# imulki/serenade

Measured on AMD Instinct MI355X. Metric: mel frames/sec converted (UNet ODE + vocoder), 80x1024, higher is better.
Workload: dtype f32

## Files before the change

serenade_amd/csrc/resunit_f32.hip:

```cpp
#include <hip/hip_runtime.h>

#include "common.h"
#include "conv_common.h"
#include "fastdiv.h"
#include "serenade_hip.h"

namespace {

constexpr int NTH = 512;

template <int C_>
struct UCfg {
  static constexpr int C = C_, CH = C / 32;
  static constexpr int BMI = C == 32 ? 256 : 128;
  static constexpr int A_ROWS = BMI + SRN_RESUNIT_HALO_MAX + 2;
  static constexpr int A_PLANE = A_ROWS * 144;
  static constexpr int A_BYTES = CH * A_PLANE;
  static constexpr int UNIT = C * 144;
  static constexpr int G = 9216 / UNIT >= 2 ? 2 : 1;
  static constexpr int STAGE = G * UNIT;
  static constexpr int SMEM = A_BYTES + 2 * STAGE;
  static constexpr int F4R = C / 4, RSTEP = NTH / F4R;
  static constexpr int A_LD = (A_ROWS * F4R + NTH - 1) / NTH;
  static_assert(G * C * 8 == NTH, "one 16-B weight piece per thread per stage");
};

template <class R, bool RAGGED = false, class... Lens>
__global__ __launch_bounds__(NTH, 4) void resunit_f32_kernel(const SrnResUnitParams p, const int tiles_per_z,
                                                             const int n_tiles, const FDiv d_tpz, const Lens... lens) {
  static_assert(sizeof...(Lens) == (RAGGED ? 1 : 0), "the ragged instance takes the lengths, the dense one nothing");
  constexpr int C = R::C, CH = R::CH, BMI = R::BMI, G = R::G;
  extern __shared__ __attribute__((aligned(16))) unsigned char smem_u[];
  unsigned char* const sA = smem_u;
  unsigned char* const sW = smem_u + R::A_BYTES;

  const int tid = threadIdx.x;
  const int lane = tid & 63;
  const int wave = __builtin_amdgcn_readfirstlane(tid >> 6);
  const int li = lane & 31;
  const int lh = lane >> 5;
  const int k = p.k, dil = p.dilation, T = p.T;
  const int p2 = (k - 1) / 2, p1 = p2 * dil;
  const int BMo = BMI - (k - 1);
  const int hr = BMI + (k - 1) * dil;
  const int U = k * CH;
  const int S = (U + G - 1) / G;
  const float slope = p.slope;
  auto item_len = [&](const int z) {
    if constexpr (RAGGED) return max(min(__builtin_amdgcn_readfirstlane(srn_first(lens...)[z]), T), 0);
    else return T;
  };

  const int w_n = (tid % (C * 8)) >> 3;
  const int w_g = tid / (C * 8);
  const int w_voff = w_n * (k * C * 4) + w_g * 128 + (tid & 7) * 16;
  const int w_dst = (w_g * C + w_n) * 144 + (tid & 7) * 16;
  const int w_bytes = C * k * C * 4;
  const __amdgpu_buffer_rsrc_t rs_w1 = srn_buffer_rsrc(p.w1, w_bytes);
  const __amdgpu_buffer_rsrc_t rs_w2 = srn_buffer_rsrc(p.w2, w_bytes);
  u32x4 wr;
  auto w_load = [&](const int j) {
    if (j >= S) wr = __builtin_amdgcn_raw_buffer_load_b128(rs_w2, w_voff, (j - S) * G * 128, 0);
    else wr = __builtin_amdgcn_raw_buffer_load_b128(rs_w1, w_voff, j * G * 128, 0);
  };
  auto w_store = [&](const int buf) {
    *reinterpret_cast<u32x4*>(sW + buf * R::STAGE + w_dst) = wr;
  };

  constexpr int A_LD = R::A_LD, F4R = R::F4R, RSTEP = R::RSTEP;
  const int a_f4 = tid % F4R;
  const int a_r0 = tid / F4R;
  const int a_voff = (a_r0 * C + a_f4 * 4) * 4;
  const int a_dst0 = (a_f4 >> 3) * R::A_PLANE + a_r0 * 144 + (a_f4 & 7) * 16;
  u32x4 pa[A_LD];
  auto load_a = [&](const int tile) {
    const int z = fdiv(tile, d_tpz);
    const int t0 = (tile - z * tiles_per_z) * BMo;
    const __amdgpu_buffer_rsrc_t rs_x = srn_buffer_rsrc(p.x + (int64_t)z * p.x_bs, item_len(z) * C * 4);
    const int v0 = a_voff + (t0 - p2 - p1) * (C * 4);
#pragma unroll
    for (int j = 0; j < A_LD; ++j) pa[j] = __builtin_amdgcn_raw_buffer_load_b128(rs_x, v0 + j * (RSTEP * C * 4), 0, 0);
  };
  auto stage_a = [&]() {
#pragma unroll
    for (int j = 0; j < A_LD; ++j) {
      if (a_r0 + RSTEP * j < hr) {
        float4 v = __builtin_bit_cast(float4, pa[j]);
        v.x = fmaxf(v.x, v.x * slope);
        v.y = fmaxf(v.y, v.y * slope);
        v.z = fmaxf(v.z, v.z * slope);
        v.w = fmaxf(v.w, v.w * slope);
        *reinterpret_cast<float4*>(sA + a_dst0 + j * RSTEP * 144) = v;
      }
    }
  };

  const int wm0 = (C == 64 ? (wave & 3) : wave) * 32;
  const int ng0 = C == 64 ? (wave >> 2) : 0;
  const int fa_lane = (wm0 + li) * 144 + 16 * lh;
  const int fb_lane = R::A_BYTES + (ng0 * 32 + li) * 144 + 16 * lh;
  f32x16 acc;
  auto zero_acc = [&]() {
#pragma unroll
    for (int r = 0; r < 16; ++r) acc[r] = 0.f;
  };

  auto compute = [&](const int buf, const int u0, const int step) {
#pragma unroll
    for (int g = 0; g < G; ++g) {
      const int u = u0 + g;
      if (u >= U) break;
      const int tap = u / CH;
      const int c = u - tap * CH;
      const float* a = reinterpret_cast<const float*>(smem_u + (fa_lane + (c * R::A_PLANE + tap * step * 144)));
      const float* b = reinterpret_cast<const float*>(smem_u + (fb_lane + (buf * R::STAGE + g * C * 144)));
#pragma unroll
      for (int kk = 0; kk < 4; ++kk) {
        const float4 af = *reinterpret_cast<const float4*>(a + kk * 8);
        const float4 bf = *reinterpret_cast<const float4*>(b + kk * 8);
        acc = __builtin_amdgcn_mfma_f32_32x32x2f32(af.x, bf.x, acc, 0, 0, 0);
        acc = __builtin_amdgcn_mfma_f32_32x32x2f32(af.y, bf.y, acc, 0, 0, 0);
        acc = __builtin_amdgcn_mfma_f32_32x32x2f32(af.z, bf.z, acc, 0, 0, 0);
        acc = __builtin_amdgcn_mfma_f32_32x32x2f32(af.w, bf.w, acc, 0, 0, 0);
      }
    }
  };

  int wj = 0, wbuf = 0;
  auto conv_pass = [&](const int step) {
    for (int s = 0; s < S; ++s) {
      compute(wbuf, s * G, step);
      w_store(wbuf ^ 1);
      int nxt = wj + 2;
      if (nxt >= 2 * S) nxt -= 2 * S;
      w_load(nxt);
      wj = wj + 1 == 2 * S ? 0 : wj + 1;
      wbuf ^= 1;
      __syncthreads();
    }
  };

  int tile = blockIdx.x;
  load_a(tile);
  w_load(0);
  w_store(0);
  w_load(2 * S > 1 ? 1 : 0);

  const float bias1 = p.b1[ng0 * 32 + li];
  const float bias2 = p.b2[ng0 * 32 + li];
  const bool divide = p.post_div != 0.f && p.post_div != 1.f;
  const bool has_q = p.res2 != nullptr;
  const int mid_lane = ng0 * R::A_PLANE + ((wm0 + 4 * lh) * 36 + li) * 4;
  const int io_lane = ((wm0 + 4 * lh) * C + ng0 * 32 + li) * 4;

  for (; tile < n_tiles; tile += gridDim.x) {
    const int z = fdiv(tile, d_tpz);
    const int t0 = (tile - z * tiles_per_z) * BMo;
    const int Tz = item_len(z);
    stage_a();
    __syncthreads();
    const int next = tile + gridDim.x;
    load_a(next < n_tiles ? next : tile);

    zero_acc();
    conv_pass(dil);
    if (t0 - p2 >= 0 && t0 - p2 + BMI <= Tz) {
#pragma unroll
      for (int r = 0; r < 16; ++r) {
        const float v = acc[r] + bias1;
        *reinterpret_cast<float*>(sA + mid_lane + ((r & 3) + 8 * (r >> 2)) * 144) = fmaxf(v, v * slope);
      }
    } else {
#pragma unroll
      for (int r = 0; r < 16; ++r) {
        const int dr = (r & 3) + 8 * (r >> 2);
        const int gi = t0 - p2 + wm0 + 4 * lh + dr;
        float v = acc[r] + bias1;
        v = fmaxf(v, v * slope);
        if (gi < 0 || gi >= Tz) v = 0.f;
        *reinterpret_cast<float*>(sA + mid_lane + dr * 144) = v;
      }
    }
    __syncthreads();

    zero_acc();
    conv_pass(1);

    const int row_end = RAGGED ? max(min(BMo, Tz - t0), 0) : min(BMo, T - t0);
    const int64_t zoff = (int64_t)t0 * C;
    const int io_bytes = row_end * C * 4;
    const __amdgpu_buffer_rsrc_t rs_xe = srn_buffer_rsrc(p.x + (int64_t)z * p.x_bs + zoff, io_bytes);
    const __amdgpu_buffer_rsrc_t rs_qe =
        srn_buffer_rsrc(has_q ? p.res2 + (int64_t)z * p.res2_bs + zoff : p.x, has_q ? io_bytes : 0);
    const __amdgpu_buffer_rsrc_t rs_oe = srn_buffer_rsrc(p.out + (int64_t)z * p.out_bs + zoff, io_bytes);
    if (wm0 + 32 <= row_end) {
#pragma unroll
      for (int gq = 0; gq < 4; ++gq) {
        float xv[4], qv[4];
#pragma unroll
        for (int i = 0; i < 4; ++i) {
          xv[i] = __builtin_bit_cast(float, __builtin_amdgcn_raw_buffer_load_b32(rs_xe, io_lane, (8 * gq + i) * C * 4, 0));
          qv[i] = __builtin_bit_cast(float, __builtin_amdgcn_raw_buffer_load_b32(rs_qe, io_lane, (8 * gq + i) * C * 4, 0));
        }
#pragma unroll
        for (int i = 0; i < 4; ++i) {
          float v = acc[4 * gq + i] + bias2 + xv[i];
          if (has_q) v += qv[i];
          if (divide) v = v / p.post_div;
          __builtin_amdgcn_raw_buffer_store_b32(__builtin_bit_cast(unsigned, v), rs_oe, io_lane, (8 * gq + i) * C * 4, 0);
        }
      }
    } else if (wm0 < row_end) {
#pragma unroll
      for (int gq = 0; gq < 4; ++gq) {
        float xv[4], qv[4];
#pragma unroll
        for (int i = 0; i < 4; ++i) {
          xv[i] = __builtin_bit_cast(float, __builtin_amdgcn_raw_buffer_load_b32(rs_xe, io_lane + (8 * gq + i) * C * 4, 0, 0));
          qv[i] = __builtin_bit_cast(float, __builtin_amdgcn_raw_buffer_load_b32(rs_qe, io_lane + (8 * gq + i) * C * 4, 0, 0));
        }
#pragma unroll
        for (int i = 0; i < 4; ++i) {
          float v = acc[4 * gq + i] + bias2 + xv[i];
          if (has_q) v += qv[i];
          if (divide) v = v / p.post_div;
          __builtin_amdgcn_raw_buffer_store_b32(__builtin_bit_cast(unsigned, v), rs_oe, io_lane + (8 * gq + i) * C * 4, 0, 0);
        }
      }
    }
  }
}

template <class R>
int launch_unit(const SrnResUnitParams& p, const SrnResUnitRoute& r, const int32_t* lens, hipStream_t stream) {
  static_assert(R::BMI == srn_resunit_bmi(R::C), "the route's tile height is the kernel's");
  if (lens) {
    static SrnSmemAttr smem_attr_ragged;
    if (const int e = smem_attr_ragged.ensure(reinterpret_cast<const void*>(&resunit_f32_kernel<R, true, SrnLens>),
                                              R::SMEM))
      return e;
    hipLaunchKernelGGL((resunit_f32_kernel<R, true, SrnLens>), dim3(r.grid), dim3(NTH), R::SMEM, stream, p, r.tiles_per_z,
                       r.n_tiles, make_fdiv((uint32_t)r.tiles_per_z), lens);
  } else {
    static SrnSmemAttr smem_attr;
    if (const int e = smem_attr.ensure(reinterpret_cast<const void*>(&resunit_f32_kernel<R>), R::SMEM)) return e;
    hipLaunchKernelGGL((resunit_f32_kernel<R>), dim3(r.grid), dim3(NTH), R::SMEM, stream, p, r.tiles_per_z, r.n_tiles,
                       make_fdiv((uint32_t)r.tiles_per_z));
  }
  SRN_CHECK_LAUNCH();
  return 0;
}

}

bool srn_resunit_f32_eligible(const SrnResUnitParams& p, const SrnResUnitRoute& r) {
  if (!(p.slope >= 0.f && p.slope <= 1.f)) return false;
  if ((int64_t)p.T * p.C * 4 >= 0x7fffffffll) return false;
  return r.n_tiles < (1 << 26);
}

int srn_resunit_f32_launch(const SrnResUnitParams& p, const SrnResUnitRoute& r, const int32_t* lens, hipStream_t stream) {
  return p.C == 32 ? launch_unit<UCfg<32>>(p, r, lens, stream) : launch_unit<UCfg<64>>(p, r, lens, stream);
}
```

Baseline: 62150.

## Assign contiguous time spans per block and carry conv halo between tiles

Each block now walks a contiguous span of time rows instead of strided independent tiles. Consecutive tiles reuse the intermediate activation halo through a register carry, which drops the recomputed (k-1)-row overlap on every tile after the first. Waves whose rows are out of range skip the MFMA compute, and the wave-to-row/column mapping for C=64 changes. The cost is sequential dependence within a span and possible load imbalance when the number of spans is small. The new span arithmetic also relies on T and the grid/batch split being correct for ragged lengths.

Result: no change. 62350, median of 6 (+0.3%).

```diff
diff --git a/serenade_amd/csrc/resunit_f32.hip b/serenade_amd/csrc/resunit_f32.hip
--- a/serenade_amd/csrc/resunit_f32.hip
+++ b/serenade_amd/csrc/resunit_f32.hip
@@ -26,8 +26,9 @@
 };
 
 template <class R, bool RAGGED = false, class... Lens>
-__global__ __launch_bounds__(NTH, 4) void resunit_f32_kernel(const SrnResUnitParams p, const int tiles_per_z,
-                                                             const int n_tiles, const FDiv d_tpz, const Lens... lens) {
+__global__ __launch_bounds__(NTH, 4) void resunit_f32_kernel(const SrnResUnitParams p, const int nz, const int q,
+                                                             const int rem, const int n_spans, const FDiv d_nz,
+                                                             const Lens... lens) {
   static_assert(sizeof...(Lens) == (RAGGED ? 1 : 0), "the ragged instance takes the lengths, the dense one nothing");
   constexpr int C = R::C, CH = R::CH, BMI = R::BMI, G = R::G;
   extern __shared__ __attribute__((aligned(16))) unsigned char smem_u[];
@@ -73,11 +74,26 @@
   const int a_voff = (a_r0 * C + a_f4 * 4) * 4;
   const int a_dst0 = (a_f4 >> 3) * R::A_PLANE + a_r0 * 144 + (a_f4 & 7) * 16;
   u32x4 pa[A_LD];
-  auto load_a = [&](const int tile) {
-    const int z = fdiv(tile, d_tpz);
-    const int t0 = (tile - z * tiles_per_z) * BMo;
-    const __amdgpu_buffer_rsrc_t rs_x = srn_buffer_rsrc(p.x + (int64_t)z * p.x_bs, item_len(z) * C * 4);
-    const int v0 = a_voff + (t0 - p2 - p1) * (C * 4);
+  struct Tile {
+    int sp, z, t0, s1;
+    bool first;
+  };
+  auto span_start = [&](const int sp) {
+    const int z = fdiv(sp, d_nz);
+    const int j = sp - z * nz;
+    const int s0 = j * q + min(j, rem);
+    return Tile{sp, z, s0, s0 + q + (j < rem ? 1 : 0), true};
+  };
+  auto next_tile = [&](const Tile& c) {
+    const int t1 = c.t0 + (c.first ? BMo : BMI);
+    if (t1 < c.s1) return Tile{c.sp, c.z, t1, c.s1, false};
+    const int sp = c.sp + (int)gridDim.x;
+    return sp < n_spans ? span_start(sp) : Tile{n_spans, c.z, c.t0, c.s1, c.first};
+  };
+  auto mid_row0 = [&](const Tile& c) { return c.first ? c.t0 - p2 : c.t0 + p2; };
+  auto load_a = [&](const Tile& c) {
+    const __amdgpu_buffer_rsrc_t rs_x = srn_buffer_rsrc(p.x + (int64_t)c.z * p.x_bs, item_len(c.z) * C * 4);
+    const int v0 = a_voff + (mid_row0(c) - p1) * (C * 4);
 #pragma unroll
     for (int j = 0; j < A_LD; ++j) pa[j] = __builtin_amdgcn_raw_buffer_load_b128(rs_x, v0 + j * (RSTEP * C * 4), 0, 0);
   };
@@ -95,8 +111,8 @@
     }
   };
 
-  const int wm0 = (C == 64 ? (wave & 3) : wave) * 32;
-  const int ng0 = C == 64 ? (wave >> 2) : 0;
+  const int wm0 = (C == 64 ? (wave >> 1) : wave) * 32;
+  const int ng0 = C == 64 ? (wave & 1) : 0;
   const int fa_lane = (wm0 + li) * 144 + 16 * lh;
   const int fb_lane = R::A_BYTES + (ng0 * 32 + li) * 144 + 16 * lh;
   f32x16 acc;
@@ -127,9 +143,9 @@
   };
 
   int wj = 0, wbuf = 0;
-  auto conv_pass = [&](const int step) {
+  auto conv_pass = [&](const int step, const bool live) {
     for (int s = 0; s < S; ++s) {
-      compute(wbuf, s * G, step);
+      if (live) compute(wbuf, s * G, step);
       w_store(wbuf ^ 1);
       int nxt = wj + 2;
       if (nxt >= 2 * S) nxt -= 2 * S;
@@ -140,8 +156,8 @@
     }
   };
 
-  int tile = blockIdx.x;
-  load_a(tile);
+  Tile cur = span_start(blockIdx.x);
+  load_a(cur);
   w_load(0);
   w_store(0);
   w_load(2 * S > 1 ? 1 : 0);
@@ -152,41 +168,48 @@
   const bool has_q = p.res2 != nullptr;
   const int mid_lane = ng0 * R::A_PLANE + ((wm0 + 4 * lh) * 36 + li) * 4;
   const int io_lane = ((wm0 + 4 * lh) * C + ng0 * 32 + li) * 4;
-
-  for (; tile < n_tiles; tile += gridDim.x) {
-    const int z = fdiv(tile, d_tpz);
-    const int t0 = (tile - z * tiles_per_z) * BMo;
+  const bool carries = a_r0 < k - 1;
+  u32x4 carry = {0u, 0u, 0u, 0u};
+
+  while (cur.sp < n_spans) {
+    const int z = cur.z, t0 = cur.t0;
+    const bool first = cur.first;
     const int Tz = item_len(z);
+    const int full = first ? BMo : BMI;
+    const int row_end = max(min(full, min(cur.s1, Tz) - t0), 0);
+    const int m0 = mid_row0(cur);
+    const int mid_off = first ? 0 : (k - 1) * 144;
     stage_a();
     __syncthreads();
-    const int next = tile + gridDim.x;
-    load_a(next < n_tiles ? next : tile);
+    const Tile nxt = next_tile(cur);
+    load_a(nxt.sp < n_spans ? nxt : cur);
 
     zero_acc();
-    conv_pass(dil);
-    if (t0 - p2 >= 0 && t0 - p2 + BMI <= Tz) {
+    conv_pass(dil, wm0 < row_end + (first ? k - 1 : 0));
+    if (m0 >= 0 && m0 + BMI <= Tz) {
 #pragma unroll
       for (int r = 0; r < 16; ++r) {
         const float v = acc[r] + bias1;
-        *reinterpret_cast<float*>(sA + mid_lane + ((r & 3) + 8 * (r >> 2)) * 144) = fmaxf(v, v * slope);
+        *reinterpret_cast<float*>(sA + mid_off + mid_lane + ((r & 3) + 8 * (r >> 2)) * 144) = fmaxf(v, v * slope);
       }
     } else {
 #pragma unroll
       for (int r = 0; r < 16; ++r) {
         const int dr = (r & 3) + 8 * (r >> 2);
-        const int gi = t0 - p2 + wm0 + 4 * lh + dr;
+        const int gi = m0 + wm0 + 4 * lh + dr;
         float v = acc[r] + bias1;
         v = fmaxf(v, v * slope);
         if (gi < 0 || gi >= Tz) v = 0.f;
-        *reinterpret_cast<float*>(sA + mid_lane + dr * 144) = v;
-      }
-    }
+        *reinterpret_cast<float*>(sA + mid_off + mid_lane + dr * 144) = v;
+      }
+    }
+    if (!first && carries) *reinterpret_cast<u32x4*>(sA + a_dst0) = carry;
     __syncthreads();
+    if (carries) carry = *reinterpret_cast<const u32x4*>(sA + a_dst0 + full * 144);
 
     zero_acc();
-    conv_pass(1);
-
-    const int row_end = RAGGED ? max(min(BMo, Tz - t0), 0) : min(BMo, T - t0);
+    conv_pass(1, wm0 < row_end);
+
     const int64_t zoff = (int64_t)t0 * C;
     const int io_bytes = row_end * C * 4;
     const __amdgpu_buffer_rsrc_t rs_xe = srn_buffer_rsrc(p.x + (int64_t)z * p.x_bs + zoff, io_bytes);
@@ -228,24 +251,29 @@
         }
       }
     }
+    cur = nxt;
   }
 }
 
 template <class R>
 int launch_unit(const SrnResUnitParams& p, const SrnResUnitRoute& r, const int32_t* lens, hipStream_t stream) {
   static_assert(R::BMI == srn_resunit_bmi(R::C), "the route's tile height is the kernel's");
+  const int nz = r.grid / p.n_batch > 1 ? r.grid / p.n_batch : 1;
+  const int n_spans = p.n_batch * nz;
+  const int grid = r.grid < n_spans ? r.grid : n_spans;
+  const int q = p.T / nz, rem = p.T % nz;
+  const FDiv d_nz = make_fdiv((uint32_t)nz);
   if (lens) {
     static SrnSmemAttr smem_attr_ragged;
     if (const int e = smem_attr_ragged.ensure(reinterpret_cast<const void*>(&resunit_f32_kernel<R, true, SrnLens>),
                                               R::SMEM))
       return e;
-    hipLaunchKernelGGL((resunit_f32_kernel<R, true, SrnLens>), dim3(r.grid), dim3(NTH), R::SMEM, stream, p, r.tiles_per_z,
-                       r.n_tiles, make_fdiv((uint32_t)r.tiles_per_z), lens);
+    hipLaunchKernelGGL((resunit_f32_kernel<R, true, SrnLens>), dim3(grid), dim3(NTH), R::SMEM, stream, p, nz, q, rem,
+                       n_spans, d_nz, lens);
   } else {
     static SrnSmemAttr smem_attr;
     if (const int e = smem_attr.ensure(reinterpret_cast<const void*>(&resunit_f32_kernel<R>), R::SMEM)) return e;
-    hipLaunchKernelGGL((resunit_f32_kernel<R>), dim3(r.grid), dim3(NTH), R::SMEM, stream, p, r.tiles_per_z, r.n_tiles,
-                       make_fdiv((uint32_t)r.tiles_per_z));
+    hipLaunchKernelGGL((resunit_f32_kernel<R>), dim3(grid), dim3(NTH), R::SMEM, stream, p, nz, q, rem, n_spans, d_nz);
   }
   SRN_CHECK_LAUNCH();
   return 0;
```
